# Tarekbouamer/Image-Retrieval-for-Image-Based-Localization

Measured on AMD Instinct MI355X. Metric: images/sec extract + queries/sec 1M-desc kNN, ResNet50-GeM 1024×768, higher is better.
Workload: dtype fp16

## Files before the change

image-retrieval-for-image-based-localization_amd/csrc/rr_c3pair.hip:

```cpp
#include "rr_internal.h"

#ifndef C3P_IG2
#define C3P_IG2 1
#endif

namespace rr {

namespace {

typedef __attribute__((ext_vector_type(4))) float cf32x4_t;
typedef __attribute__((ext_vector_type(4))) int ci32x4_t;

constexpr unsigned COOB = 0x80000000u;

__device__ __forceinline__ void cdma16(ci32x4_t rsrc, unsigned voff, unsigned lds_addr) {
    unsigned keep;
    lds_addr = __builtin_amdgcn_readfirstlane(lds_addr);
    asm volatile(
        "s_mov_b32 %0, m0\n\t"
        "s_mov_b32 m0, %3\n\t"
        "s_nop 0\n\t"
        "buffer_load_dwordx4 %1, %2, 0 offen lds\n\t"
        "s_mov_b32 m0, %0"
        : "=&s"(keep)
        : "v"(voff), "s"(rsrc), "s"(lds_addr)
        : "memory");
}

__device__ __forceinline__ ci32x4_t crsrc(const void* base, unsigned bytes) {
    const unsigned long long b = (unsigned long long)base;
    ci32x4_t r;
    r.x = __builtin_amdgcn_readfirstlane((int)(unsigned)b);
    r.y = __builtin_amdgcn_readfirstlane((int)((unsigned)(b >> 32) & 0xFFFFu));
    r.z = __builtin_amdgcn_readfirstlane((int)bytes);
    r.w = 0x00020000;
    int x = r.x, y = r.y, z = r.z;
    asm volatile("s_nop 4" : "+s"(x), "+s"(y), "+s"(z));
    r.x = x;
    r.y = y;
    r.z = z;
    return r;
}

__device__ __forceinline__ void cbar() { asm volatile("s_waitcnt lgkmcnt(0)\n\ts_barrier" ::: "memory"); }

template <int K>
__device__ __forceinline__ int cwswz(int row, int chunk) {
    const int f = K == 64 ? ((row >> 1) & 7) : (row & 15);
    return row * (K * 2) + ((chunk ^ f) << 4);
}

__device__ __forceinline__ void cpin(uint4& v) { asm volatile("" : "+v"(v.x), "+v"(v.y), "+v"(v.z), "+v"(v.w)); }

}

struct C3PairArgs {
    const bf16_t* t1;
    const bf16_t* w0;
    const float *s0, *h0;
    const bf16_t* w33;
    const float *s33, *h33;
    const bf16_t* w3;
    const float *s3, *h3;
    const bf16_t* res;
    const bf16_t* xp;
    const bf16_t* wp;
    const float *sp, *hp;
    const bf16_t* w1;
    const float *s1, *h1;
    bf16_t* y;
    bf16_t* z;
    int* queue;
    int n, h, w;
    int act2, act3, act1, act0;
    float slope2, slope3, slope1, slope0;
};

namespace {

template <int C1, bool PROJ, typename HT, bool CONV1 = false>
__global__ void __launch_bounds__(512, 1) k_c3pair(C3PairArgs a, int tiles_w, int tiles_hw, int ntiles) {
    static_assert(!CONV1 || PROJ, "conv1 in the launch: the stage's first block only");
    constexpr int TH = 4, TW = 32, TP = TH * TW, PITCH = 40;
    constexpr int NSLOT = (TH + 2) * PITCH, NP = NSLOT / 8;
    constexpr int PCW = TW + 2;
    constexpr int FN = 4;
    constexpr int K3 = 64, C3 = 256, NK3 = K3 / 32, NR3 = C3 / 32, NF1 = C1 / 16, NK1 = C3 / 32;
    static_assert(NSLOT % 8 == 0 && PITCH % 8 == 0, "row-invariant patch swizzle");
    __shared__ __attribute__((aligned(1024))) char sPatch[NSLOT * 128];
    __shared__ __attribute__((aligned(16))) char sT2[TP * 128];
    __shared__ __attribute__((aligned(16))) char sW3[C3 * K3 * 2];
    __shared__ __attribute__((aligned(16))) char sW1[C1 * C3 * 2];
    __shared__ __attribute__((aligned(16))) char sWp[PROJ ? C3 * K3 * 2 : 16];
    __shared__ __attribute__((aligned(16))) float sS3[C3], sH3[C3], sS1[C1], sH1[C1], sS2[64], sH2[64];
    __shared__ __attribute__((aligned(16))) float sSp[PROJ ? C3 : 4], sHp[PROJ ? C3 : 4];
    __shared__ __attribute__((aligned(16))) char sW0[CONV1 ? 64 * 64 * 2 : 16];
    __shared__ __attribute__((aligned(16))) float sS0[CONV1 ? 64 : 4], sH0[CONV1 ? 64 : 4];
    __shared__ int sTile[4];

    const int tid = threadIdx.x, lane = tid & 63;
    const int wave = __builtin_amdgcn_readfirstlane(tid >> 6);
    const bool role3 = wave < 4;
    const int r16 = lane & 15, kq = lane >> 4, lrow = lane >> 3, lch = lane & 7;
    const int H = a.h, W = a.w;

    for (int i = tid; i < C3 * K3 / 8; i += 512) {
        const int r = i / (K3 / 8), c = i - r * (K3 / 8);
        *reinterpret_cast<uint4*>(sW3 + cwswz<K3>(r, c)) = reinterpret_cast<const uint4*>(a.w3)[i];
        if constexpr (PROJ) *reinterpret_cast<uint4*>(sWp + cwswz<K3>(r, c)) = reinterpret_cast<const uint4*>(a.wp)[i];
    }
    for (int i = tid; i < C1 * C3 / 8; i += 512) {
        const int r = i / (C3 / 8), c = i - r * (C3 / 8);
        *reinterpret_cast<uint4*>(sW1 + cwswz<C3>(r, c)) = reinterpret_cast<const uint4*>(a.w1)[i];
    }
    for (int i = tid; i < C3; i += 512) {
        sS3[i] = a.s3[i];
        sH3[i] = a.h3[i];
        if constexpr (PROJ) {
            sSp[i] = a.sp[i];
            sHp[i] = a.hp[i];
        }
    }
    for (int i = tid; i < C1; i += 512) {
        sS1[i] = a.s1[i];
        sH1[i] = a.h1[i];
    }
    if (tid < 64) {
        sS2[tid] = a.s33[tid];
        sH2[tid] = a.h33[tid];
        if constexpr (CONV1) {
            sS0[tid] = a.s0[tid];
            sH0[tid] = a.h0[tid];
        }
    }
    if constexpr (CONV1)
        for (int i = tid; i < 64 * 64 / 8; i += 512) {
            const int r = i / 8, c = i - r * 8;
            *reinterpret_cast<uint4*>(sW0 + cwswz<64>(r, c)) = reinterpret_cast<const uint4*>(a.w0)[i];
        }
    const int wc = wave & 1, wpx = (wave >> 1) & 1;

    const int b = (int)blockIdx.x, G = (int)gridDim.x, xcd = b & 7;
    const int nt8 = ntiles >> 3, rt8 = ntiles & 7;
    const int s_x = xcd < rt8 ? xcd * (nt8 + 1) : rt8 * (nt8 + 1) + (xcd - rt8) * nt8;
    const int n_x = nt8 + (xcd < rt8 ? 1 : 0);
    auto fetch_tile = [&](int i) __attribute__((always_inline)) {
        if (a.queue) {
            const int v = atomicAdd(a.queue + xcd, 1);
            return v < n_x ? s_x + v : -1;
        }
        const int t = i * G + xcd * (G >> 3) + (b >> 3);
        return t < ntiles ? t : -1;
    };
    if (tid == 0) {
        sTile[0] = fetch_tile(0);
        sTile[1] = fetch_tile(1);
        sTile[2] = fetch_tile(2);
    }
    __syncthreads();
    auto tile_id = [&](int i) __attribute__((always_inline)) { return sTile[i & 3]; };
    if (tile_id(0) < 0) return;
    auto tile_org = [&](int t, int& img, int& oh0, int& ow0) __attribute__((always_inline)) {
        img = t / tiles_hw;
        const int rem = t - img * tiles_hw, th = rem / tiles_w;
        oh0 = th * TH;
        ow0 = (rem - th * tiles_w) * TW;
    };

    const ci32x4_t rsX = crsrc(a.t1, (unsigned)((long long)a.n * H * W * 64 * 2));
    const unsigned ldsP = (unsigned)(unsigned long long)sPatch;
    auto patch_dma = [&](int t, bool live) __attribute__((always_inline)) {
        int img = 0, oh0 = 0, ow0 = 0;
        if (live) tile_org(t, img, oh0, ow0);
        int lr = lrow;
        asm volatile("" : "+v"(lr));
#pragma unroll
        for (int u = 0; u < 8; ++u) {
            const int d = wave + 4 * u, q = d * 8 + lr;
            if (d >= NP) break;
            const int pr = q / PITCH, pc = q - pr * PITCH;
            const int hh = oh0 - 1 + pr, ww = ow0 - 1 + pc;
            unsigned off = COOB;
            if (live && pc < PCW && (unsigned)hh < (unsigned)H && (unsigned)ww < (unsigned)W)
                off = (unsigned)(((((long long)img * H + hh) * W + ww) * 64 + ((lch ^ lr) << 3)) * 2);
            cdma16(rsX, off, ldsP + d * 1024);
        }
    };
    h16_f32x4_t acc[2][FN];
    auto conv3x3 = [&](const uint4 (&areg)[2][18]) __attribute__((always_inline)) {
        int lc;
        asm volatile("v_mbcnt_lo_u32_b32 %0, -1, 0\n\tv_mbcnt_hi_u32_b32 %0, -1, %0" : "=v"(lc));
        lc &= 15;
        const char* base[FN][3][2];
#pragma unroll
        for (int j = 0; j < FN; ++j)
#pragma unroll
            for (int dx = 0; dx < 3; ++dx)
#pragma unroll
                for (int hs = 0; hs < 2; ++hs) {
                    const int q = (wpx * 2 + (j >> 1)) * PITCH + (j & 1) * 16 + lc + dx;
                    base[j][dx][hs] = sPatch + q * 128 + (((kq + 4 * hs) ^ (q & 7)) << 4);
                }
#pragma unroll
        for (int ii = 0; ii < 2; ++ii)
#pragma unroll
            for (int j = 0; j < FN; ++j) acc[ii][j] = (h16_f32x4_t){0.f, 0.f, 0.f, 0.f};
#pragma unroll
        for (int s = 0; s < 18; ++s) {
            const int tap = s >> 1, hs = s & 1, dy = tap / 3, dx = tap % 3;
            uint4 fb[FN];
#pragma unroll
            for (int j = 0; j < FN; ++j) fb[j] = *reinterpret_cast<const uint4*>(base[j][dx][hs] + dy * PITCH * 128);
#pragma unroll
            for (int ii = 0; ii < 2; ++ii)
#pragma unroll
                for (int j = 0; j < FN; ++j) acc[ii][j] = H16<HT>::mfma(areg[ii][s], fb[j], acc[ii][j]);
        }
    };
    auto convert_patch = [&](int t) __attribute__((always_inline)) {
        if constexpr (CONV1) {
            int img, oh0, ow0;
            tile_org(t, img, oh0, ow0);
            const bool leaky0 = a.act0 == RR_ACT_LEAKY;
            for (int f = wave; f < NP * 8 / 16; f += 4) {
                int q = f * 16 + r16;
                asm volatile("" : "+v"(q));
                const int pr = q / PITCH, pc = q - pr * PITCH;
                const int hh = oh0 - 1 + pr, ww = ow0 - 1 + pc;
                const bool valid = pc < PCW && (unsigned)hh < (unsigned)H && (unsigned)ww < (unsigned)W;
                char* slot = sPatch + q * 128;
                uint4 bx[2];
#pragma unroll
                for (int kk = 0; kk < 2; ++kk)
                    bx[kk] = *reinterpret_cast<const uint4*>(slot + (((4 * kk + kq) ^ (q & 7)) << 4));
                h16_f32x4_t c0[4];
#pragma unroll
                for (int ii = 0; ii < 4; ++ii) c0[ii] = (h16_f32x4_t){0.f, 0.f, 0.f, 0.f};
#pragma unroll
                for (int kk = 0; kk < 2; ++kk)
#pragma unroll
                    for (int ii = 0; ii < 4; ++ii) {
                        const uint4 av = *reinterpret_cast<const uint4*>(sW0 + cwswz<64>(ii * 16 + r16, kk * 4 + kq));
                        c0[ii] = H16<HT>::mfma(av, bx[kk], c0[ii]);
                    }
#pragma unroll
                for (int i2 = 0; i2 < 2; ++i2) {
                    const int c = 32 * i2 + 8 * kq;
                    float v[8];
#pragma unroll
                    for (int r = 0; r < 4; ++r) {
                        v[r] = c0[2 * i2][r] * sS0[c + r] + sH0[c + r];
                        v[4 + r] = c0[2 * i2 + 1][r] * sS0[c + 4 + r] + sH0[c + 4 + r];
                    }
                    if (leaky0) {
#pragma unroll
                        for (int r = 0; r < 8; ++r) v[r] = v[r] > 0.f ? v[r] : v[r] * a.slope0;
                    }
                    uint4 o = make_uint4(0u, 0u, 0u, 0u);
                    if (valid) {
                        o.x = H16<HT>::pack2(v[0], v[1]);
                        o.y = H16<HT>::pack2(v[2], v[3]);
                        o.z = H16<HT>::pack2(v[4], v[5]);
                        o.w = H16<HT>::pack2(v[6], v[7]);
                    }
                    *reinterpret_cast<uint4*>(slot + (((4 * i2 + kq) ^ (q & 7)) << 4)) = o;
                }
            }
        }
    };
    auto store_t2 = [&]() __attribute__((always_inline)) {
        const int c = 32 * wc + 8 * kq;
        float sc[8], sh[8];
#pragma unroll
        for (int r = 0; r < 8; ++r) {
            sc[r] = sS2[c + r];
            sh[r] = sH2[c + r];
        }
        const bool leaky2 = a.act2 == RR_ACT_LEAKY;
#pragma unroll
        for (int j = 0; j < FN; ++j) {
            const int p = wpx * (TP / 2) + j * 16 + r16;
            float v[8];
#pragma unroll
            for (int r = 0; r < 4; ++r) {
                v[r] = acc[0][j][r] * sc[r] + sh[r];
                v[4 + r] = acc[1][j][r] * sc[4 + r] + sh[4 + r];
            }
            if (leaky2) {
#pragma unroll
                for (int r = 0; r < 8; ++r) v[r] = v[r] > 0.f ? v[r] : v[r] * a.slope2;
            }
            uint4 o;
            o.x = H16<HT>::pack2(v[0], v[1]);
            o.y = H16<HT>::pack2(v[2], v[3]);
            o.z = H16<HT>::pack2(v[4], v[5]);
            o.w = H16<HT>::pack2(v[6], v[7]);
            *reinterpret_cast<uint4*>(sT2 + p * 128 + (((4 * wc + kq) ^ (p & 7)) << 4)) = o;
        }
    };

    const int pw = wave - 4;
    const bool leaky3 = a.act3 == RR_ACT_LEAKY, leaky1 = a.act1 == RR_ACT_LEAKY;
    constexpr int NRQ = PROJ ? NK3 : NR3;
    auto strip_pixel = [&](int t, int k) __attribute__((always_inline)) {
        int img, oh0, ow0;
        tile_org(t, img, oh0, ow0);
        return ((long long)img * H + oh0 + (k >> 1)) * W + ow0 + (k & 1) * 16 + r16;
    };
    auto load_rq = [&](uint4 (&dst)[NRQ], long long p) __attribute__((always_inline)) {
        if constexpr (PROJ) {
            const bf16_t* ps = a.xp + p * K3 + 8 * kq;
#pragma unroll
            for (int kk = 0; kk < NK3; ++kk) dst[kk] = ld16_once(ps + kk * 32);
        } else {
            const bf16_t* rs = a.res + p * C3 + 8 * kq;
#pragma unroll
            for (int i2 = 0; i2 < NR3; ++i2) dst[i2] = ld16_once(rs + 32 * i2);
        }
    };
    auto pair_strip = [&](int k, long long p, const uint4 (&rv)[NRQ]) __attribute__((always_inline)) {
        uint4 bq[NK3];
        {
            const int q = k * 16 + r16;
#pragma unroll
            for (int kk = 0; kk < NK3; ++kk)
                bq[kk] = *reinterpret_cast<const uint4*>(sT2 + q * 128 + (((4 * kk + kq) ^ (q & 7)) << 4));
        }
        uint4 yq[NR3];
        constexpr int IG = C3P_IG2 ? 2 : 1;
#pragma unroll
        for (int i0 = 0; i0 < NR3; i0 += IG) {
            int abase = 0;
            asm volatile("" : "+v"(abase));
            h16_f32x4_t acc3[IG][2], pacc[IG][2];
#pragma unroll
            for (int g = 0; g < IG; ++g)
#pragma unroll
                for (int hh = 0; hh < 2; ++hh) acc3[g][hh] = pacc[g][hh] = (h16_f32x4_t){0.f, 0.f, 0.f, 0.f};
#pragma unroll
            for (int kk = 0; kk < NK3; ++kk)
#pragma unroll
                for (int g = 0; g < IG; ++g)
#pragma unroll
                    for (int hh = 0; hh < 2; ++hh) {
                        const uint4 av = *reinterpret_cast<const uint4*>(sW3 + abase + cwswz<K3>((2 * (i0 + g) + hh) * 16 + r16, kk * 4 + kq));
                        acc3[g][hh] = H16<HT>::mfma(av, bq[kk], acc3[g][hh]);
                    }
            if constexpr (PROJ) {
#pragma unroll
                for (int kk = 0; kk < NK3; ++kk)
#pragma unroll
                    for (int g = 0; g < IG; ++g)
#pragma unroll
                        for (int hh = 0; hh < 2; ++hh) {
                            const uint4 av = *reinterpret_cast<const uint4*>(sWp + abase + cwswz<K3>((2 * (i0 + g) + hh) * 16 + r16, kk * 4 + kq));
                            pacc[g][hh] = H16<HT>::mfma(av, rv[kk], pacc[g][hh]);
                        }
            }
#pragma unroll
            for (int g = 0; g < IG; ++g) {
                const int i2 = i0 + g;
                const int c = 32 * i2 + 8 * kq;
                float v[8];
#pragma unroll
                for (int r = 0; r < 4; ++r) {
                    v[r] = acc3[g][0][r] * sS3[c + r] + sH3[c + r];
                    v[4 + r] = acc3[g][1][r] * sS3[c + 4 + r] + sH3[c + 4 + r];
                }
                if constexpr (PROJ) {
#pragma unroll
                    for (int r = 0; r < 4; ++r) {
                        v[r] += pacc[g][0][r] * sSp[c + r] + sHp[c + r];
                        v[4 + r] += pacc[g][1][r] * sSp[c + 4 + r] + sHp[c + 4 + r];
                    }
                } else {
                    const uint4 qv = rv[i2];
                    const unsigned w4[4] = {qv.x, qv.y, qv.z, qv.w};
#pragma unroll
                    for (int r = 0; r < 4; ++r) {
                        v[2 * r] += H16<HT>::lo(w4[r]);
                        v[2 * r + 1] += H16<HT>::hi(w4[r]);
                    }
                }
                if (leaky3) {
#pragma unroll
                    for (int r = 0; r < 8; ++r) v[r] = v[r] > 0.f ? v[r] : v[r] * a.slope3;
                }
                yq[i2].x = H16<HT>::pack2(v[0], v[1]);
                yq[i2].y = H16<HT>::pack2(v[2], v[3]);
                yq[i2].z = H16<HT>::pack2(v[4], v[5]);
                yq[i2].w = H16<HT>::pack2(v[6], v[7]);
                st16_once(a.y + p * C3 + c, yq[i2]);
            }
        }
        h16_f32x4_t zacc[NF1];
#pragma unroll
        for (int o = 0; o < NF1; ++o) zacc[o] = (h16_f32x4_t){0.f, 0.f, 0.f, 0.f};
#pragma unroll
        for (int kk = 0; kk < NK1; ++kk) {
            int abase = 0;
            asm volatile("" : "+v"(abase));
#pragma unroll
            for (int o = 0; o < NF1; ++o) {
                const uint4 av = *reinterpret_cast<const uint4*>(sW1 + abase + cwswz<C3>(o * 16 + r16, kk * 4 + kq));
                zacc[o] = H16<HT>::mfma(av, yq[kk], zacc[o]);
            }
        }
#pragma unroll
        for (int o2 = 0; o2 < NF1 / 2; ++o2) {
            const int c = 32 * o2 + 8 * kq;
            float v[8];
#pragma unroll
            for (int r = 0; r < 4; ++r) {
                v[r] = zacc[2 * o2][r] * sS1[c + r] + sH1[c + r];
                v[4 + r] = zacc[2 * o2 + 1][r] * sS1[c + 4 + r] + sH1[c + 4 + r];
            }
            if (leaky1) {
#pragma unroll
                for (int r = 0; r < 8; ++r) v[r] = v[r] > 0.f ? v[r] : v[r] * a.slope1;
            }
            uint4 o;
            o.x = H16<HT>::pack2(v[0], v[1]);
            o.y = H16<HT>::pack2(v[2], v[3]);
            o.z = H16<HT>::pack2(v[4], v[5]);
            o.w = H16<HT>::pack2(v[6], v[7]);
            st16_once(a.z + p * C1 + c, o);
        }
    };

    if (role3) {
        uint4 areg[2][18];
#pragma unroll
        for (int i = 0; i < 2; ++i)
#pragma unroll
            for (int ks = 0; ks < 18; ++ks)
                areg[i][ks] = *reinterpret_cast<const uint4*>(a.w33 + (long long)(32 * wc + 16 * i + r16) * 576 +
                                                              (ks >> 1) * 64 + 32 * (ks & 1) + 8 * kq);
#pragma unroll
        for (int i = 0; i < 2; ++i)
#pragma unroll
            for (int ks = 0; ks < 18; ++ks) cpin(areg[i][ks]);
        auto conv = [&]() __attribute__((always_inline)) { conv3x3(areg); };
        patch_dma(tile_id(0), true);
        asm volatile("s_waitcnt vmcnt(0)" ::: "memory");
        cbar();
        if constexpr (CONV1) {
            convert_patch(tile_id(0));
            cbar();
        }
        conv();
        if (wpx == 0) store_t2();
        cbar();
        patch_dma(tile_id(1), tile_id(1) >= 0);
        asm volatile("s_waitcnt vmcnt(0)" ::: "memory");
        cbar();
        for (int s = 0; tile_id(s) >= 0; ++s) {
            const bool more = tile_id(s + 1) >= 0;
            if (wpx == 1) store_t2();
            if constexpr (CONV1) {
                if (more) convert_patch(tile_id(s + 1));
                cbar();
            }
            if (more) conv();
            cbar();
            if (more) {
                if (wpx == 0) store_t2();
                const int t2i = tile_id(s + 2);
                patch_dma(t2i, t2i >= 0);
                if (tid == 0) sTile[(s + 3) & 3] = t2i >= 0 ? fetch_tile(s + 3) : -1;
                asm volatile("s_waitcnt vmcnt(0)" ::: "memory");
            }
            cbar();
        }
    } else {
        __builtin_amdgcn_s_setprio(1);
        uint4 rq[4][NRQ];
        load_rq(rq[0], strip_pixel(tile_id(0), pw));
        load_rq(rq[1], strip_pixel(tile_id(0), 4 + pw));
        cbar();
        if constexpr (CONV1) cbar();
        cbar();
        cbar();
        for (int s = 0; tile_id(s) >= 0; s += 2) {
            {
                const int t = tile_id(s);
                const bool n1 = tile_id(s + 1) >= 0;
                if (n1) load_rq(rq[2], strip_pixel(tile_id(s + 1), pw));
                if constexpr (CONV1) cbar();
                pair_strip(pw, strip_pixel(t, pw), rq[0]);
                cbar();
                if (n1) load_rq(rq[3], strip_pixel(tile_id(s + 1), 4 + pw));
                pair_strip(4 + pw, strip_pixel(t, 4 + pw), rq[1]);
                cbar();
            }
            if (tile_id(s + 1) >= 0) {
                const int t = tile_id(s + 1);
                const bool n2 = tile_id(s + 2) >= 0;
                if (n2) load_rq(rq[0], strip_pixel(tile_id(s + 2), pw));
                if constexpr (CONV1) cbar();
                pair_strip(pw, strip_pixel(t, pw), rq[2]);
                cbar();
                if (n2) load_rq(rq[1], strip_pixel(tile_id(s + 2), 4 + pw));
                pair_strip(4 + pw, strip_pixel(t, 4 + pw), rq[3]);
                cbar();
            }
        }
    }
}

}

}

using namespace rr;

extern "C" int rr_conv3x3_pair(const void* t1, int n, int h, int w, const void* w0, const float* scale0,
                               const float* shift0, int act0, float slope0, const void* w33, const float* scale2,
                               const float* shift2, int act2, float slope2, const void* w3, const float* scale3,
                               const float* shift3, const void* residual, const void* xp, const void* wp,
                               const float* scalep, const float* shiftp, int act3, float slope3, const void* w1,
                               const float* scale1, const float* shift1, int c_out, int act1, float slope1, void* y,
                               void* z, int* tile_queue, int dtype, void* stream) {
    if (dtype != RR_BF16 && dtype != RR_F16) return fail(RR_EINVAL, "rr_conv3x3_pair: dtype (bf16 / fp16)");
    if (!t1 || !w33 || !scale2 || !shift2 || !w3 || !scale3 || !shift3 || !w1 || !scale1 || !shift1 || !y || !z)
        return fail(RR_EINVAL, "rr_conv3x3_pair: null pointer");
    const bool proj = residual == nullptr;
    if (proj && (!xp || !wp || !scalep || !shiftp))
        return fail(RR_EINVAL, "rr_conv3x3_pair: either residual or the projection (xp, wp, scalep, shiftp)");
    if (c_out != 64 && c_out != 128) return fail(RR_EINVAL, "rr_conv3x3_pair: c_out 64 or 128");
    if (proj && c_out != 64) return fail(RR_EINVAL, "rr_conv3x3_pair: the projection form takes c_out = 64");
    const bool conv1 = w0 != nullptr;
    if (conv1 && (!proj || !scale0 || !shift0 || ((uintptr_t)w0 & 15)))
        return fail(RR_EINVAL, "rr_conv3x3_pair: conv1 in the launch (w0) needs the projection form, scale0, shift0");
    if (conv1 && act0 != RR_ACT_IDENTITY && act0 != RR_ACT_LEAKY) return fail(RR_EINVAL, "rr_conv3x3_pair: act0");
    if (n <= 0 || h <= 0 || w <= 0 || h % 4 || w % 32) return fail(RR_EINVAL, "rr_conv3x3_pair: h % 4, w % 32");
    if ((long long)n * h * w * 64 * 2 >= (1ll << 31)) return fail(RR_EINVAL, "rr_conv3x3_pair: t1 over 2 GiB (split the batch)");
    for (const void* p : {t1, w33, w3, residual, xp, wp, w1, (const void*)y, (const void*)z})
        if ((uintptr_t)p & 15) return fail(RR_EINVAL, "rr_conv3x3_pair: 16-byte alignment required");
    if ((uintptr_t)tile_queue & 3) return fail(RR_EINVAL, "rr_conv3x3_pair: tile_queue alignment");
    for (int act : {act2, act3, act1})
        if (act != RR_ACT_IDENTITY && act != RR_ACT_LEAKY) return fail(RR_EINVAL, "rr_conv3x3_pair: activation");
    C3PairArgs a;
    a.t1 = (const bf16_t*)t1; a.w33 = (const bf16_t*)w33; a.s33 = scale2; a.h33 = shift2;
    a.w3 = (const bf16_t*)w3; a.s3 = scale3; a.h3 = shift3; a.res = (const bf16_t*)residual;
    a.xp = (const bf16_t*)xp; a.wp = (const bf16_t*)wp; a.sp = scalep; a.hp = shiftp;
    a.w1 = (const bf16_t*)w1; a.s1 = scale1; a.h1 = shift1; a.y = (bf16_t*)y; a.z = (bf16_t*)z;
    a.n = n; a.h = h; a.w = w; a.act2 = act2; a.act3 = act3; a.act1 = act1;
    a.slope2 = slope2; a.slope3 = slope3; a.slope1 = slope1; a.queue = tile_queue;
    a.w0 = (const bf16_t*)w0; a.s0 = scale0; a.h0 = shift0; a.act0 = act0; a.slope0 = slope0;
    const int tiles_w = w / 32, tiles_hw = (h / 4) * tiles_w;
    const long long ntl = (long long)n * tiles_hw;
    if (ntl >= (1ll << 31)) return fail(RR_EINVAL, "rr_conv3x3_pair: too many tiles");
    const int cus = grid_cus();
    int grid = (int)(ntl < cus ? ntl : cus) & ~7;
    if (grid < 8) grid = 8;
    const dim3 g((unsigned)grid), b(512);
    hipStream_t s = as_stream(stream);
    auto go = [&](auto hv) {
        using H = decltype(hv);
        if (conv1) hipLaunchKernelGGL((k_c3pair<64, true, H, true>), g, b, 0, s, a, tiles_w, tiles_hw, (int)ntl);
        else if (proj) hipLaunchKernelGGL((k_c3pair<64, true, H>), g, b, 0, s, a, tiles_w, tiles_hw, (int)ntl);
        else if (c_out == 64) hipLaunchKernelGGL((k_c3pair<64, false, H>), g, b, 0, s, a, tiles_w, tiles_hw, (int)ntl);
        else hipLaunchKernelGGL((k_c3pair<128, false, H>), g, b, 0, s, a, tiles_w, tiles_hw, (int)ntl);
    };
    if (dtype == RR_F16) go(f16_t{});
    else go(bf16_t{});
    return check_launch("rr_conv3x3_pair");
}
```

Before: 5638.

## Keep projection weight fragments in registers and relax address barriers in c3pair

For the non-conv1 projection launch, the first 9 of 16 Wp row blocks are loaded once into per-lane registers of the pair waves, so their MFMA A-operands come from registers instead of LDS, and the shared Wp buffer shrinks to match. The empty asm that blocks hoisting of the LDS address base becomes non-volatile and takes the strip pixel as input, which lets the compiler schedule the weight loads more freely. Optional timestamp instrumentation on barriers is added behind a compile flag. The register-resident fragments add a lot of VGPR pressure in a kernel launched with a 512-thread bound, which risks spills.

After: 5665, median of 6. About the same (+0.5%).

```diff
diff --git a/image-retrieval-for-image-based-localization_amd/csrc/rr_c3pair.hip b/image-retrieval-for-image-based-localization_amd/csrc/rr_c3pair.hip
--- a/image-retrieval-for-image-based-localization_amd/csrc/rr_c3pair.hip
+++ b/image-retrieval-for-image-based-localization_amd/csrc/rr_c3pair.hip
@@ -2,6 +2,12 @@
 
 #ifndef C3P_IG2
 #define C3P_IG2 1
+#endif
+#ifndef C3P_WFREE
+#define C3P_WFREE 1
+#endif
+#ifndef C3P_WPR_PROJ
+#define C3P_WPR_PROJ 9
 #endif
 
 namespace rr {
@@ -42,7 +48,8 @@
     return r;
 }
 
-__device__ __forceinline__ void cbar() { asm volatile("s_waitcnt lgkmcnt(0)\n\ts_barrier" ::: "memory"); }
+enum { BAR_PRO = 0, BAR_A = 1, BAR_B = 2, BAR_CV = 3 };
+__device__ __forceinline__ void cbar(int = BAR_PRO) { asm volatile("s_waitcnt lgkmcnt(0)\n\ts_barrier" ::: "memory"); }
 
 template <int K>
 __device__ __forceinline__ int cwswz(int row, int chunk) {
@@ -74,13 +81,19 @@
     int n, h, w;
     int act2, act3, act1, act0;
     float slope2, slope3, slope1, slope0;
+#ifdef C3P_STAMPS
+    unsigned long long* stamps;
+    int stamp_cap;
+#endif
 };
 
 namespace {
 
-template <int C1, bool PROJ, typename HT, bool CONV1 = false>
+template <int C1, bool PROJ, typename HT, bool CONV1 = false, int NWR = 0>
 __global__ void __launch_bounds__(512, 1) k_c3pair(C3PairArgs a, int tiles_w, int tiles_hw, int ntiles) {
     static_assert(!CONV1 || PROJ, "conv1 in the launch: the stage's first block only");
+    static_assert(NWR == 0 || PROJ, "Wp fragments in registers: the projection form only");
+    static_assert(NWR >= 0 && NWR < 16, "Wp has 16 row blocks");
     constexpr int TH = 4, TW = 32, TP = TH * TW, PITCH = 40;
     constexpr int NSLOT = (TH + 2) * PITCH, NP = NSLOT / 8;
     constexpr int PCW = TW + 2;
@@ -91,7 +104,7 @@
     __shared__ __attribute__((aligned(16))) char sT2[TP * 128];
     __shared__ __attribute__((aligned(16))) char sW3[C3 * K3 * 2];
     __shared__ __attribute__((aligned(16))) char sW1[C1 * C3 * 2];
-    __shared__ __attribute__((aligned(16))) char sWp[PROJ ? C3 * K3 * 2 : 16];
+    __shared__ __attribute__((aligned(16))) char sWp[PROJ ? (C3 - 16 * NWR) * K3 * 2 : 16];
     __shared__ __attribute__((aligned(16))) float sS3[C3], sH3[C3], sS1[C1], sH1[C1], sS2[64], sH2[64];
     __shared__ __attribute__((aligned(16))) float sSp[PROJ ? C3 : 4], sHp[PROJ ? C3 : 4];
     __shared__ __attribute__((aligned(16))) char sW0[CONV1 ? 64 * 64 * 2 : 16];
@@ -103,11 +116,24 @@
     const bool role3 = wave < 4;
     const int r16 = lane & 15, kq = lane >> 4, lrow = lane >> 3, lch = lane & 7;
     const int H = a.h, W = a.w;
+#ifdef C3P_STAMPS
+    int nst = 0;
+    unsigned long long* const stp =
+        a.stamps ? a.stamps + ((long long)blockIdx.x * 8 + wave) * a.stamp_cap : nullptr;
+    auto cbar = [&](int tag = BAR_PRO) __attribute__((always_inline)) {
+        if (stp && nst < a.stamp_cap && lane == 0) stp[nst] = ((unsigned long long)__builtin_amdgcn_s_memtime() << 2) | tag;
+        ++nst;
+        rr::cbar();
+    };
+#endif
 
     for (int i = tid; i < C3 * K3 / 8; i += 512) {
         const int r = i / (K3 / 8), c = i - r * (K3 / 8);
         *reinterpret_cast<uint4*>(sW3 + cwswz<K3>(r, c)) = reinterpret_cast<const uint4*>(a.w3)[i];
-        if constexpr (PROJ) *reinterpret_cast<uint4*>(sWp + cwswz<K3>(r, c)) = reinterpret_cast<const uint4*>(a.wp)[i];
+        if constexpr (PROJ) {
+            if (r >= 16 * NWR)
+                *reinterpret_cast<uint4*>(sWp + cwswz<K3>(r - 16 * NWR, c)) = reinterpret_cast<const uint4*>(a.wp)[i];
+        }
     }
     for (int i = tid; i < C1 * C3 / 8; i += 512) {
         const int r = i / (C3 / 8), c = i - r * (C3 / 8);
@@ -318,6 +344,7 @@
             for (int i2 = 0; i2 < NR3; ++i2) dst[i2] = ld16_once(rs + 32 * i2);
         }
     };
+    uint4 wpr[NWR ? NWR : 1][NK3];
     auto pair_strip = [&](int k, long long p, const uint4 (&rv)[NRQ]) __attribute__((always_inline)) {
         uint4 bq[NK3];
         {
@@ -331,7 +358,8 @@
 #pragma unroll
         for (int i0 = 0; i0 < NR3; i0 += IG) {
             int abase = 0;
-            asm volatile("" : "+v"(abase));
+            if constexpr (C3P_WFREE) asm("" : "+v"(abase) : "v"((int)p));
+            else asm volatile("" : "+v"(abase));
             h16_f32x4_t acc3[IG][2], pacc[IG][2];
 #pragma unroll
             for (int g = 0; g < IG; ++g)
@@ -353,7 +381,10 @@
                     for (int g = 0; g < IG; ++g)
 #pragma unroll
                         for (int hh = 0; hh < 2; ++hh) {
-                            const uint4 av = *reinterpret_cast<const uint4*>(sWp + abase + cwswz<K3>((2 * (i0 + g) + hh) * 16 + r16, kk * 4 + kq));
+                            const int rb = 2 * (i0 + g) + hh;
+                            uint4 av;
+                            if (rb < NWR) av = wpr[rb < NWR ? rb : 0][kk];
+                            else av = *reinterpret_cast<const uint4*>(sWp + abase + cwswz<K3>((rb - NWR) * 16 + r16, kk * 4 + kq));
                             pacc[g][hh] = H16<HT>::mfma(av, rv[kk], pacc[g][hh]);
                         }
             }
@@ -399,7 +430,8 @@
 #pragma unroll
         for (int kk = 0; kk < NK1; ++kk) {
             int abase = 0;
-            asm volatile("" : "+v"(abase));
+            if constexpr (C3P_WFREE) asm("" : "+v"(abase) : "v"((int)p));
+            else asm volatile("" : "+v"(abase));
 #pragma unroll
             for (int o = 0; o < NF1; ++o) {
                 const uint4 av = *reinterpret_cast<const uint4*>(sW1 + abase + cwswz<C3>(o * 16 + r16, kk * 4 + kq));
@@ -459,10 +491,10 @@
             if (wpx == 1) store_t2();
             if constexpr (CONV1) {
                 if (more) convert_patch(tile_id(s + 1));
-                cbar();
+                cbar(BAR_CV);
             }
             if (more) conv();
-            cbar();
+            cbar(BAR_A);
             if (more) {
                 if (wpx == 0) store_t2();
                 const int t2i = tile_id(s + 2);
@@ -470,13 +502,22 @@
                 if (tid == 0) sTile[(s + 3) & 3] = t2i >= 0 ? fetch_tile(s + 3) : -1;
                 asm volatile("s_waitcnt vmcnt(0)" ::: "memory");
             }
-            cbar();
+            cbar(BAR_B);
         }
     } else {
         __builtin_amdgcn_s_setprio(1);
         uint4 rq[4][NRQ];
         load_rq(rq[0], strip_pixel(tile_id(0), pw));
         load_rq(rq[1], strip_pixel(tile_id(0), 4 + pw));
+        if constexpr (NWR > 0) {
+#pragma unroll
+            for (int rb = 0; rb < NWR; ++rb)
+#pragma unroll
+                for (int kk = 0; kk < NK3; ++kk) {
+                    wpr[rb][kk] = reinterpret_cast<const uint4*>(a.wp)[(rb * 16 + r16) * (K3 / 8) + kk * 4 + kq];
+                    cpin(wpr[rb][kk]);
+                }
+        }
         cbar();
         if constexpr (CONV1) cbar();
         cbar();
@@ -486,23 +527,23 @@
                 const int t = tile_id(s);
                 const bool n1 = tile_id(s + 1) >= 0;
                 if (n1) load_rq(rq[2], strip_pixel(tile_id(s + 1), pw));
-                if constexpr (CONV1) cbar();
+                if constexpr (CONV1) cbar(BAR_CV);
                 pair_strip(pw, strip_pixel(t, pw), rq[0]);
-                cbar();
+                cbar(BAR_A);
                 if (n1) load_rq(rq[3], strip_pixel(tile_id(s + 1), 4 + pw));
                 pair_strip(4 + pw, strip_pixel(t, 4 + pw), rq[1]);
-                cbar();
+                cbar(BAR_B);
             }
             if (tile_id(s + 1) >= 0) {
                 const int t = tile_id(s + 1);
                 const bool n2 = tile_id(s + 2) >= 0;
                 if (n2) load_rq(rq[0], strip_pixel(tile_id(s + 2), pw));
-                if constexpr (CONV1) cbar();
+                if constexpr (CONV1) cbar(BAR_CV);
                 pair_strip(pw, strip_pixel(t, pw), rq[2]);
-                cbar();
+                cbar(BAR_A);
                 if (n2) load_rq(rq[1], strip_pixel(tile_id(s + 2), 4 + pw));
                 pair_strip(4 + pw, strip_pixel(t, 4 + pw), rq[3]);
-                cbar();
+                cbar(BAR_B);
             }
         }
     }
@@ -513,6 +554,16 @@
 }
 
 using namespace rr;
+
+#ifdef C3P_STAMPS
+static unsigned long long* g_c3p_stamps = nullptr;
+static int g_c3p_stamp_cap = 0;
+extern "C" int rr_c3pair_stamps(void* buf, int cap) {
+    g_c3p_stamps = (unsigned long long*)buf;
+    g_c3p_stamp_cap = cap;
+    return RR_OK;
+}
+#endif
 
 extern "C" int rr_conv3x3_pair(const void* t1, int n, int h, int w, const void* w0, const float* scale0,
                                const float* shift0, int act0, float slope0, const void* w33, const float* scale2,
@@ -548,6 +599,10 @@
     a.n = n; a.h = h; a.w = w; a.act2 = act2; a.act3 = act3; a.act1 = act1;
     a.slope2 = slope2; a.slope3 = slope3; a.slope1 = slope1; a.queue = tile_queue;
     a.w0 = (const bf16_t*)w0; a.s0 = scale0; a.h0 = shift0; a.act0 = act0; a.slope0 = slope0;
+#ifdef C3P_STAMPS
+    a.stamps = g_c3p_stamps;
+    a.stamp_cap = g_c3p_stamp_cap;
+#endif
     const int tiles_w = w / 32, tiles_hw = (h / 4) * tiles_w;
     const long long ntl = (long long)n * tiles_hw;
     if (ntl >= (1ll << 31)) return fail(RR_EINVAL, "rr_conv3x3_pair: too many tiles");
@@ -559,7 +614,8 @@
     auto go = [&](auto hv) {
         using H = decltype(hv);
         if (conv1) hipLaunchKernelGGL((k_c3pair<64, true, H, true>), g, b, 0, s, a, tiles_w, tiles_hw, (int)ntl);
-        else if (proj) hipLaunchKernelGGL((k_c3pair<64, true, H>), g, b, 0, s, a, tiles_w, tiles_hw, (int)ntl);
+        else if (proj)
+            hipLaunchKernelGGL((k_c3pair<64, true, H, false, C3P_WPR_PROJ>), g, b, 0, s, a, tiles_w, tiles_hw, (int)ntl);
         else if (c_out == 64) hipLaunchKernelGGL((k_c3pair<64, false, H>), g, b, 0, s, a, tiles_w, tiles_hw, (int)ntl);
         else hipLaunchKernelGGL((k_c3pair<128, false, H>), g, b, 0, s, a, tiles_w, tiles_hw, (int)ntl);
     };
```
